# shenyunhang/APE

Hardware: AMD Instinct MI355X
Metric: images/sec @1024^2 APE-L_D fwd (higher is better)
Workload: dtype bf16

## Files before the change

ape_amd/_lib.py:

```python
import ctypes
import os
from ctypes import POINTER, Structure, c_char_p, c_double, c_float, c_int, c_int32, c_int64, c_void_p

_HERE = os.path.dirname(os.path.abspath(__file__))
LIB_PATH = os.path.join(_HERE, "lib", "libape_hip.so")

DT_F32 = 0
DT_BF16 = 1
DT_F16 = 2
ACT_NONE, ACT_RELU, ACT_GELU, ACT_SWIGLU, ACT_SILU = 0, 1, 2, 3, 4
MASK_NONE, MASK_ZERO_INPUT, MASK_ZERO_OUTPUT = 0, 1, 2


class GemmArgs(Structure):
    _fields_ = [
        ("A", c_void_p), ("W", c_void_p), ("C", c_void_p), ("bias", c_void_p), ("residual", c_void_p),
        ("rowmask", c_void_p), ("rope_cos", c_void_p), ("rope_sin", c_void_p),
        ("M", c_int32), ("N", c_int32), ("K", c_int32),
        ("lda", c_int32), ("ldw", c_int32), ("ldc", c_int32), ("ldr", c_int32),
        ("in_dt", c_int32), ("out_dt", c_int32), ("res_dt", c_int32),
        ("act", c_int32), ("mask_mode", c_int32), ("trans_out", c_int32),
        ("rope_rows", c_int32), ("rope_hd", c_int32), ("rope_cols", c_int32), ("vec_ok", c_int32),
        ("alpha", c_float), ("clamp", c_float),
        ("splitk", c_int32), ("tile64", c_int32), ("workspace", c_void_p),
# ... 98 lines not shown
    "ape_hip_query_init": (c_int, [c_void_p, c_void_p, c_int, c_void_p, c_int, c_float, c_int, c_void_p, c_void_p, c_int, c_int, c_void_p,
                                   c_void_p]),
    "ape_hip_query_finish": (c_int, [c_void_p, c_int, c_void_p, c_int, c_int, c_int, c_void_p, c_void_p, c_float, c_void_p, c_void_p,
                                     c_float, c_void_p, c_void_p, c_void_p, c_int, c_int, c_void_p]),
    "ape_hip_bilinear_resize": (c_int, [c_void_p, c_int, c_int, c_int, c_int, c_int, c_void_p, c_int, c_int, c_void_p]),
    "ape_hip_panoptic_pixels": (c_int, [c_void_p, c_int, c_int, c_int, c_int, c_int, c_void_p, c_void_p, c_float, c_int, c_int, c_void_p, c_void_p,
                                        c_void_p, c_void_p]),
    "ape_hip_panoptic_decide": (c_int, [c_void_p, c_void_p, c_void_p, c_int, c_void_p, c_int, c_double, c_int, c_void_p, c_void_p, c_void_p, c_void_p]),
    "ape_hip_panoptic_write": (c_int, [c_void_p, c_void_p, c_void_p, c_int, c_int, c_void_p, c_void_p]),
    "ape_hip_enc_finalize": (c_int, [c_void_p, c_void_p, c_void_p, c_int, c_void_p, c_void_p, c_void_p, c_void_p]),
    "ape_hip_topk_workspace_words": (c_int, [c_int]),
    "ape_hip_proposal_topk": (c_int, [c_void_p, c_int, POINTER(c_int), POINTER(c_int), c_int, c_int, c_int, c_void_p, c_void_p, c_void_p,
                                      c_void_p]),
    "ape_hip_proposal_order": (c_int, [c_void_p, c_int, c_void_p, c_void_p, POINTER(c_int), POINTER(c_int), c_int, c_void_p, c_void_p,
                                       c_void_p, c_void_p, c_void_p, c_void_p, c_void_p]),
    "ape_hip_proposal_quota": (c_int, [c_void_p, c_void_p, c_void_p, c_void_p, c_int, c_void_p, c_int, POINTER(c_int), POINTER(c_int),
                                       c_int, c_int, c_void_p, c_void_p]),
    "ape_hip_det_sort": (c_int, [c_void_p, c_int, c_int, c_int, c_void_p, c_void_p, c_float, c_void_p, c_void_p, c_void_p, c_void_p,
                                 c_void_p, c_void_p]),
    "ape_hip_det_topk": (c_int, [c_void_p, c_void_p, c_void_p, c_void_p, c_int, c_int, c_int, c_void_p, c_void_p, c_void_p, c_void_p,
                                 c_void_p, c_void_p]),
    "ape_hip_ffn_fused": (c_int, [c_void_p, c_int, c_void_p, c_int, c_void_p, c_void_p, c_int, c_void_p, c_void_p, c_int, c_void_p, c_int,
                                  c_int, c_int, c_int, c_int, c_int, c_int, c_void_p, c_void_p, c_float, c_void_p]),
    "ape_hip_attention_ext": (c_int, [c_void_p, c_int, c_void_p, c_int, c_void_p, c_int, c_void_p, c_int, c_int, c_int, c_int, c_int, c_int,
                                      c_int, c_float, c_int, c_void_p]),
    "ape_hip_relpos_extend": (c_int, [c_void_p, c_void_p, c_int, c_void_p, c_int, c_int, c_void_p, c_void_p, c_int, c_void_p, c_void_p, c_int, c_int,
                                      c_int, c_int, c_int, c_int, c_int, c_int, c_float, c_int, c_void_p]),
    "ape_hip_resize_coeffs": (c_int, [c_int, c_int, c_void_p, c_void_p, c_int]),
    "ape_hip_resize_tile_rows": (c_int, [c_void_p, c_int, POINTER(c_int)]),
    "ape_hip_resize_bilinear_u8": (c_int, [c_void_p, c_int, c_int, c_int, c_void_p, c_void_p, c_int, c_void_p, c_void_p, c_int,
                                           c_int, c_int, c_int, c_int, c_void_p, c_int, c_int, c_int, c_int, c_void_p]),
    "ape_hip_rle_workspace_words": (c_int, [c_int, c_int, c_int, c_int]),
    "ape_hip_rle_encode": (c_int, [c_void_p, c_int, c_int, c_int, c_void_p, c_void_p, c_int, c_void_p, c_void_p]),
    "ape_hip_rle_to_string": (c_int, [c_void_p, c_int, c_void_p, c_int]),
    "ape_hip_label_hist_lds_bins": (c_int, []),
    "ape_hip_label_pair_hist": (c_int, [c_void_p, c_int, c_void_p, c_int, ctypes.c_size_t, c_int, c_int, c_int, c_int, c_void_p, c_void_p,
                                        c_void_p]),
    "ape_hip_mask_pack_bits": (c_int, [c_void_p, c_int, ctypes.c_size_t, ctypes.c_size_t, c_void_p, ctypes.c_size_t, c_void_p, c_void_p]),
    "ape_hip_mask_paired_counts": (c_int, [c_void_p, ctypes.c_size_t, c_void_p, ctypes.c_size_t, c_int, ctypes.c_size_t, c_void_p, c_void_p]),
    "ape_hip_bitmask_pair_counts": (c_int, [c_void_p, c_int, ctypes.c_size_t, c_void_p, c_int, ctypes.c_size_t, ctypes.c_size_t, c_void_p,
                                            ctypes.c_size_t, c_void_p]),
    "ape_hip_rle_decode_workspace_words": (c_int, [c_int, c_int]),
    "ape_hip_rle_decode": (c_int, [c_void_p, c_void_p, c_int, c_int, c_int, c_int, c_void_p, c_void_p, c_void_p]),
    "ape_hip_rle_from_string": (c_int, [c_void_p, c_int, c_void_p, c_int]),
    "ape_hip_mask_pack_rows": (c_int, [c_void_p, c_int, c_int, c_int, c_void_p, ctypes.c_size_t, c_void_p, c_void_p]),
    "ape_hip_bitmask_boundary": (c_int, [c_void_p, c_int, c_int, c_int, c_int, ctypes.c_size_t, c_void_p, ctypes.c_size_t, c_void_p,
# ... 35 lines not shown
```

ape_amd/csrc/ffn_fused.hip:

```cpp
#include <stdlib.h>

#include "common.h"
#include "../../include/ape_hip.h"

typedef __attribute__((address_space(3))) void ff_lds_void_t;
typedef const __attribute__((address_space(1))) void ff_gbl_void_t;

#define FF_K 256
#define FF_HC 64
#define FF_N 256
#define FF_BM 128
#define FF_STAGE 65536

struct FfnParams {
  const bf16_t* X; int ldx;
  const bf16_t* W1; int ldw1;
  const float* b1;
  const bf16_t* W2; int ldw2;
  const float* b2;
  const bf16_t* R; int ldr;
  bf16_t* Y; int ldy;
  int M, HID;
  const float* ln_w; const float* ln_b; float ln_eps;
};

__device__ __forceinline__ float ff_rows_sum(float v) {
  const unsigned u = __float_as_uint(v);
  const auto a = __builtin_amdgcn_permlane16_swap(u, u, false, false);
  const float m = __uint_as_float(a[0]) + __uint_as_float(a[1]);
  const unsigned w = __float_as_uint(m);
  const auto b = __builtin_amdgcn_permlane32_swap(w, w, false, false);
  return __uint_as_float(b[0]) + __uint_as_float(b[1]);
}

template <bool W2P, int RT, typename H = bf16_t>
__global__ __launch_bounds__(256, 1) void ffn_fused_kernel(const FfnParams p) {
  extern __shared__ __attribute__((aligned(16))) unsigned char smem[];
  float* sb1 = reinterpret_cast<float*>(smem + 2 * FF_STAGE);
  float* sb2 = sb1 + p.HID;
  const int tid = threadIdx.x, lane = tid & 63, wave = tid >> 6;
  const int fm = lane & 15, g = lane >> 4;
  const int row0 = blockIdx.x * (64 * RT) + wave * (16 * RT);

  for (int i = tid; i < p.HID; i += 256) sb1[i] = p.b1[i];
  for (int i = tid; i < FF_N; i += 256) sb2[i] = p.b2[i];

  bf16x8_t xf[RT][8];
  int tok[RT];
#pragma unroll
  for (int rt = 0; rt < RT; ++rt) {
    tok[rt] = row0 + rt * 16 + fm;
    const bf16_t* xp = p.X + (size_t)(tok[rt] < p.M ? tok[rt] : p.M - 1) * p.ldx + g * 8;
#pragma unroll
    for (int ks = 0; ks < 8; ++ks) xf[rt][ks] = __builtin_bit_cast(bf16x8_t, *reinterpret_cast<const short8_t*>(xp + ks * 32));
  }

  uint32_t w1off[8], w2off[8];
#pragma unroll
// ... 125 lines not shown
#define FF_DMA(J) issue_piece(cn, s ^ 1, (J)); FF_SB();
    rd1(0, fa); rd1(1, fb); FF_SB();
    rd1(2, fc); mm1(0, fa); FF_MIX(8); FF_SB(); FF_DMA(0)
    rd1(3, fa); act(0); mm1(1, fb); FF_MIX(8); FF_SB(); FF_DMA(1)
    rd2(0, 0, fb); act(1); pack(0); mm1(2, fc); FF_MIX(8); FF_SB(); FF_DMA(2)
    rd2(0, 1, fc); act(2); mm1(3, fa); FF_MIX(8); FF_SB(); FF_DMA(3)
    rd2(1, 0, fa); act(3); pack(1); mm2(0, 0, fb); FF_MIX(8); FF_SB(); FF_DMA(4)
    rd2(1, 1, fb); mm2(0, 1, fc); FF_MIX(8); FF_SB(); FF_DMA(5)
    mm2(1, 0, fa); FF_SB(); FF_DMA(6)
    FF_DMA(7)
    mm2(1, 1, fb); FF_SB();
#undef FF_DMA
#undef FF_MIX
#undef FF_SB
    asm volatile("s_waitcnt vmcnt(0)" ::: "memory");
    __syncthreads();
  }

#pragma unroll
  for (int rt = 0; rt < RT; ++rt) {
    const int tk = tok[rt] < p.M ? tok[rt] : p.M - 1;
    const bf16_t* rp = p.R != nullptr ? p.R + (size_t)tk * p.ldr + g * 8 : nullptr;
    float v[64];
#pragma unroll
    for (int q = 0; q < 8; ++q) {
      const float4 ba = *reinterpret_cast<const float4*>(sb2 + q * 32 + g * 8);
      const float4 bb = *reinterpret_cast<const float4*>(sb2 + q * 32 + g * 8 + 4);
      v[q * 8 + 0] = yacc[2 * q][rt][0] + ba.x; v[q * 8 + 1] = yacc[2 * q][rt][1] + ba.y;
      v[q * 8 + 2] = yacc[2 * q][rt][2] + ba.z; v[q * 8 + 3] = yacc[2 * q][rt][3] + ba.w;
      v[q * 8 + 4] = yacc[2 * q + 1][rt][0] + bb.x; v[q * 8 + 5] = yacc[2 * q + 1][rt][1] + bb.y;
      v[q * 8 + 6] = yacc[2 * q + 1][rt][2] + bb.z; v[q * 8 + 7] = yacc[2 * q + 1][rt][3] + bb.w;
      if (rp != nullptr) {
        float r[8];
        ld8<H>(reinterpret_cast<const H*>(rp + q * 32), r);
#pragma unroll
        for (int e = 0; e < 8; ++e) v[q * 8 + e] += r[e];
      }
    }
    if (p.ln_w != nullptr) {
      float sum = 0.f;
#pragma unroll
      for (int e = 0; e < 64; ++e) sum += v[e];
      const float mean = ff_rows_sum(sum) * (1.f / FF_N);
      float d2 = 0.f;
#pragma unroll
      for (int e = 0; e < 64; ++e) { v[e] -= mean; d2 = fmaf(v[e], v[e], d2); }
      const float rstd = rsqrtf(ff_rows_sum(d2) * (1.f / FF_N) + p.ln_eps);
#pragma unroll
      for (int q = 0; q < 16; ++q) {
        const float4 w = *reinterpret_cast<const float4*>(p.ln_w + (q >> 1) * 32 + g * 8 + (q & 1) * 4);
        const float4 b = *reinterpret_cast<const float4*>(p.ln_b + (q >> 1) * 32 + g * 8 + (q & 1) * 4);
        v[q * 4 + 0] = fmaf(v[q * 4 + 0] * rstd, w.x, b.x); v[q * 4 + 1] = fmaf(v[q * 4 + 1] * rstd, w.y, b.y);
        v[q * 4 + 2] = fmaf(v[q * 4 + 2] * rstd, w.z, b.z); v[q * 4 + 3] = fmaf(v[q * 4 + 3] * rstd, w.w, b.w);
      }
    }
    if (tok[rt] < p.M) {
      bf16_t* yp = p.Y + (size_t)tok[rt] * p.ldy + g * 8;
#pragma unroll
      for (int q = 0; q < 8; ++q) st8<H>(reinterpret_cast<H*>(yp + q * 32), v + q * 8);
    }
  }
}

extern "C" int ape_hip_ffn_fused(const void* X, int ldx, const void* W1, int ldw1, const float* b1, const void* W2, int ldw2, const float* b2,
                                 const void* residual, int ldr, void* Y, int ldy, int M, int K, int HID, int N, int w2_permuted, int dt,
                                 const float* ln_weight, const float* ln_bias, float ln_eps, void* stream) {
  APE_CHECK_ARG(X && W1 && b1 && W2 && b2 && Y && M > 0, "ape_hip_ffn_fused: null pointer / empty problem");
  APE_CHECK_ARG(ape_is16(dt), "ape_hip_ffn_fused: dt must be APE_DT_BF16 or APE_DT_F16 (got %d)", dt);
  APE_CHECK_ARG(K == FF_K && N == FF_N && HID % FF_HC == 0 && HID >= FF_HC && HID <= 4096,
                "ape_hip_ffn_fused: the kernel is built for 256 -> HID -> 256 with HID %% 64 == 0, HID <= 4096 (got %d -> %d -> %d)", K, HID, N);
  APE_CHECK_ARG(ldx % 8 == 0 && ldw1 % 8 == 0 && ldw2 % 8 == 0 && ldy % 8 == 0 && (residual == nullptr || ldr % 8 == 0),
                "ape_hip_ffn_fused: leading dimensions must be multiples of 8");
  APE_CHECK_ARG(((uintptr_t)X) % 16 == 0 && ((uintptr_t)W1) % 16 == 0 && ((uintptr_t)W2) % 16 == 0 && ((uintptr_t)Y) % 16 == 0 &&
                    ((uintptr_t)residual) % 16 == 0 && ((uintptr_t)b1) % 16 == 0 && ((uintptr_t)b2) % 16 == 0,
                "ape_hip_ffn_fused: 16-byte aligned pointers");
  APE_CHECK_ARG((size_t)HID * ldw1 * 2 < (1ull << 32) && (size_t)FF_N * ldw2 * 2 < (1ull << 32), "ape_hip_ffn_fused: weights too large for 32-bit offsets");
  FfnParams p;
  p.X = (const bf16_t*)X; p.ldx = ldx; p.W1 = (const bf16_t*)W1; p.ldw1 = ldw1; p.b1 = b1; p.W2 = (const bf16_t*)W2; p.ldw2 = ldw2; p.b2 = b2;
  p.R = (const bf16_t*)residual; p.ldr = ldr; p.Y = (bf16_t*)Y; p.ldy = ldy; p.M = M; p.HID = HID;
  APE_CHECK_ARG((ln_weight == nullptr) == (ln_bias == nullptr) && ((uintptr_t)ln_weight) % 16 == 0 && ((uintptr_t)ln_bias) % 16 == 0,
                "ape_hip_ffn_fused: LayerNorm weight and bias come together, 16-byte aligned");
  p.ln_w = ln_weight; p.ln_b = ln_bias; p.ln_eps = ln_eps;
  const size_t lds = 2 * FF_STAGE + (size_t)(HID + FF_N) * sizeof(float);
  const char* rt_env = getenv("APE_FFN_RT");
  const int rt = rt_env != nullptr ? atoi(rt_env) : (ceil_div(M, 192) >= 256 ? 3 : 2);
#define FF_LAUNCH(W2P_, RT_, H_)                                                                                              \
  do {                                                                                                                        \
    static ApeOncePerDevice attr__;                                                                                               \
    if (attr__.first()) {                                                                                                            \
      (void)hipFuncSetAttribute((const void*)ffn_fused_kernel<W2P_, RT_, H_>, hipFuncAttributeMaxDynamicSharedMemorySize, 160 * 1024); \
    }                                                                                                                         \
    APE_LAUNCH((ffn_fused_kernel<W2P_, RT_, H_>), dim3(ceil_div(M, 64 * RT_)), dim3(256), lds, (hipStream_t)stream, p); \
  } while (0)
  if (dt == APE_DT_F16) {
    if (w2_permuted && rt == 3) FF_LAUNCH(true, 3, f16_t); else if (w2_permuted) FF_LAUNCH(true, 2, f16_t); else FF_LAUNCH(false, 2, f16_t);
  } else {
    if (w2_permuted && rt == 3) FF_LAUNCH(true, 3, bf16_t); else if (w2_permuted) FF_LAUNCH(true, 2, bf16_t); else FF_LAUNCH(false, 2, bf16_t);
  }
#undef FF_LAUNCH
  APE_CHECK_LAUNCH("ffn_fused_kernel");
  return 0;
}
```

ape_amd/layers/fuse_helper.py:

```python
import torch
import torch.nn as nn

from .. import ops
from ..packing import attach_cache, f32, ln_params, pack_matrix


class BiMultiHeadAttention(nn.Module):
    def __init__(self, v_dim, l_dim, embed_dim, num_heads, dropout=0.1, stable_softmax_2d=False,
                 clamp_min_for_underflow=True, clamp_max_for_overflow=True, use_attention_mask_v=False):
        super().__init__()
        self.embed_dim, self.num_heads, self.head_dim = embed_dim, num_heads, embed_dim // num_heads
        self.v_dim, self.l_dim = v_dim, l_dim
        assert self.head_dim * num_heads == embed_dim
        self.scale = self.head_dim ** (-0.5)
        self.dropout = dropout
        self.v_proj = nn.Linear(v_dim, embed_dim)
        self.l_proj = nn.Linear(l_dim, embed_dim)
        self.values_v_proj = nn.Linear(v_dim, embed_dim)
        self.values_l_proj = nn.Linear(l_dim, embed_dim)
        self.out_v_proj = nn.Linear(embed_dim, v_dim)
        self.out_l_proj = nn.Linear(embed_dim, l_dim)
        self.stable_softmax_2d = stable_softmax_2d
        self.clamp_min_for_underflow = clamp_min_for_underflow
        self.clamp_max_for_overflow = clamp_max_for_overflow
# ... 70 lines not shown
        gmax = S.max().reshape(1)
        pv = ops.segment_softmax(S, nh, gmax, dt)
        v_new = ops.gemm(pv, Zt, Pd["bov"], residual=v_n, out_dtype=dt)
        qp = v_new + lvl_pos
        plT = ops.col_softmax_t(S, gmax, dt, pad=8)
        vT = ops.transpose(v_n, pad=8)
        G = ops.gemm(plT, vT, None, out_dtype=dt)
        ol = torch.empty((L, nh * hd), dtype=dt, device=dev)
        for h in range(nh):
            ops.gemm(G[h * L:(h + 1) * L], Pd["wvv"][h], Pd["bvv"][h], out=ol[:, h * hd:(h + 1) * hd])
        dl = ops.gemm(ol, Pd["wol"], Pd["bol"], out_dtype=torch.float32)
        l_new = l_n + P["gl"] * dl
        return v_new, qp, l_new

    def forward_tokens(self, x, lvl_pos, l, dt, defer_language=False):
        if l.shape[0] == 1:
            v_new, qp, ljob = self.forward_tokens_single(x, lvl_pos, l, dt)
        else:
            v_new, qp, l_new = self.forward_tokens_dense(x, lvl_pos, l, dt)
            ljob = ops._Joined(l_new)
        return (v_new, qp, ljob) if defer_language else (v_new, qp, ljob.join())

    def forward_tokens_single(self, x, lvl_pos, l, dt):
        P = self.packed(dt)
        a = self.attn
        l_n = ops.layernorm(l, P["lnl"][0], P["lnl"][1], P["lnl"][2], out_dtype=torch.float32)
        k = ops.gemv(l_n, P["wl"], P["bl"])
        vl = ops.gemv(l_n, P["wvl"], P["bvl"])
        gdv, lnb = ops.gemv(vl, P["wov"], P["bov"], scale=P["gv"], add=P["lnv"][1][None, :])
        v_new, qp = ops.layernorm(x, P["lnv"][0], lnb[0], P["lnv"][2], out_dtype=dt, add=lvl_pos)

        def language_side():
            kh = k.view(a.num_heads, a.head_dim)
            u, u_c = ops.head_gemv(kh, P["wvT"], bf16_copy=dt if dt in ops.HALF16 else True)
            c = ops.head_gemv(kh, P["bv1"], alpha=a.scale)
            _, sbias = ops.gemv(gdv, u, alpha=-a.scale, add=c.view(1, -1))
            S = ops.gemm(v_new, u_c if dt in ops.HALF16 else u, sbias[0], alpha=a.scale, out_dtype=torch.float32)
            pooled = ops.vl_pool(S, v_new, gdv[0])
            ol = ops.head_gemv(pooled, P["wvv"], P["bvv"])
            return ops.gemv(ol.view(1, -1), P["wol"], P["bol"], scale=P["gl"], add=l_n)[1]

        return v_new, qp, ops.fork(language_side)

    def forward(self, v, l, attention_mask_v=None, attention_mask_l=None):
        if attention_mask_l is not None:
            raise NotImplementedError("ape_amd BiAttentionBlock: per-token language masks (un-reduced expression tokens, "
                                      "text_feature_reduce_before_fusion=False) are not implemented")
        dt = getattr(self, "compute_dtype", torch.bfloat16)
        vs, ls = [], []
        for b in range(v.shape[0]):
            zeros = torch.zeros_like(v[b], dtype=dt)
            vn, _, ln = self.forward_tokens(v[b].to(dt).contiguous(), zeros, l[b].float().contiguous(), dt)
            vs.append(vn.to(v.dtype))
            ls.append(ln.to(l.dtype))
        return torch.stack(vs), torch.stack(ls)
```

ape_amd/modeling/ape_deta/_containers.py:

```python
import os

import torch
import torch.nn as nn

from ... import ops
from ...packing import attach_cache, f32, ln_params, pack_matrix, permute_ffn_w2


class FFN(nn.Module):
    def __init__(self, embed_dim=256, feedforward_dim=1024, output_dim=None, num_fcs=2, ffn_drop=0.0, **kwargs):
        super().__init__()
        assert num_fcs == 2
        output_dim = embed_dim if output_dim is None else output_dim
        self.layers = nn.Sequential(nn.Sequential(nn.Linear(embed_dim, feedforward_dim), nn.ReLU(inplace=True), nn.Dropout(ffn_drop)),
                                    nn.Linear(feedforward_dim, output_dim), nn.Dropout(ffn_drop))
        self.embed_dim = embed_dim
        attach_cache(self)

    def packed(self, dt):
        def build(dt):
            l0, l1 = self.layers[0][0], self.layers[1]
            d = dict(w1=pack_matrix(l0.weight, dt), b1=f32(l0.bias), w2=pack_matrix(l1.weight, dt), b2=f32(l1.bias))
            if dt in ops.HALF16 and l0.weight.shape[0] % 64 == 0:
                d["w2p"] = permute_ffn_w2(d["w2"])
            return d
        return self._pack.get(self, dt, build)

    FUSED_MIN_ROWS = 2048

    def forward_tokens(self, x, dt, out_dtype=None, norm=None):
        P = self.packed(dt)
        mode = os.environ.get("APE_FFN_FUSED", "1")
        if (mode != "0" and "w2p" in P and (out_dtype or dt) in ops.HALF16 and (out_dtype or dt) == dt and x.shape[0] >= self.FUSED_MIN_ROWS
                and x.shape[1] == 256 and P["w2"].shape[0] == 256 and P["w1"].shape[0] <= 4096):
            fuse_ln = norm if os.environ.get("APE_FFN_LN") != "0" else None
            if mode == "b64":
                y = ops.ffn_fused(x, P["w1"], P["b1"], P["w2"], P["b2"], residual=x, norm=fuse_ln)
            else:
                y = ops.ffn_fused(x, P["w1"], P["b1"], P["w2p"], P["b2"], residual=x, w2_permuted=True, norm=fuse_ln)
            return y if (norm is None or fuse_ln is not None) else ops.layernorm(y, norm[0], norm[1], norm[2], out_dtype=dt)
        h = ops.gemm(x, P["w1"], P["b1"], act=ops.ACT_RELU)
        y = ops.gemm(h, P["w2"], P["b2"], residual=x, out_dtype=out_dtype or dt)
        return y if norm is None else ops.layernorm(y, norm[0], norm[1], norm[2], out_dtype=dt)


class MLP(nn.Module):
    def __init__(self, input_dim, hidden_dim, output_dim, num_layers):
        super().__init__()
        self.num_layers = num_layers
        h = [hidden_dim] * (num_layers - 1)
        self.layers = nn.ModuleList(nn.Linear(n, k) for n, k in zip([input_dim] + h, h + [output_dim]))
        attach_cache(self)

    def packed(self, dt):
        def build(dt):
            return [(pack_matrix(l.weight, dt), f32(l.bias)) for l in self.layers]
        return self._pack.get(self, dt, build)
# ... 78 lines not shown
```

ape_amd/modeling/ape_deta/deformable_transformer_vl.py:

```python
import copy

import torch
import torch.nn as nn

from ... import ops
from ...layers import MultiScaleDeformableAttention
from ...packing import attach_cache, f32, ln_params, pack_matrix, round_up
from ...stagetap import forcing, tap
from . import geometry as G
from ._containers import FFN, SelfAttention, TransformerLayer


class DeformableDetrTransformerEncoderVL(nn.Module):
    def __init__(self, embed_dim=256, num_heads=8, feedforward_dim=1024, attn_dropout=0.1, ffn_dropout=0.1, num_layers=6,
                 post_norm=False, num_feature_levels=4, vl_layer=None, use_act_checkpoint=False, pytorch_attn=False):
        super().__init__()
        self.layers = nn.ModuleList([
            TransformerLayer([MultiScaleDeformableAttention(embed_dim=embed_dim, num_heads=num_heads, dropout=attn_dropout,
                                                            batch_first=True, num_levels=num_feature_levels,
                                                            pytorch_attn=pytorch_attn)],
                             FFN(embed_dim=embed_dim, feedforward_dim=feedforward_dim, output_dim=embed_dim, num_fcs=2,
                                 ffn_drop=ffn_dropout), 2, embed_dim) for _ in range(num_layers)])
        self.num_layers = num_layers
        self.embed_dim = embed_dim
        self.pre_norm = False
        self.post_norm_layer = nn.LayerNorm(embed_dim) if post_norm else None
        self.vl_layers = nn.ModuleList([copy.deepcopy(vl_layer) for _ in range(num_layers)]) if vl_layer is not None else None
        self.use_checkpoint = use_act_checkpoint

    def forward_tokens(self, x, geo, lvl_pos, l, dt, stages=None):
        xp = None
        for i, layer in enumerate(self.layers):
            if self.vl_layers is None:
                v_new, qp, ljob = x, (xp if xp is not None else (x.float() + lvl_pos.float()).to(dt)), ops._Joined(l)
            else:
                v_new, qp, ljob = self.vl_layers[i].b_attn.forward_tokens(x, lvl_pos, l, dt, defer_language=True)
            x2 = layer.attentions[0].forward_tokens(qp, v_new, geo.enc_ref, geo.shapes, geo.starts, dt, value_src=v_new,
                                                    mask=geo.mask_u8, norm=layer.norm_params(0))
            x, xp = layer.ffns[0].forward_tokens(x2, dt, norm=layer.norm_params(1)), None
            l = ljob.join()
            if stages is not None:
                if self.vl_layers is not None:
                    stages[f"enc{i}_fused_v"] = v_new
                    l = tap(stages, f"enc{i}_fused_l", l)
                x = tap(stages, f"enc{i}_out", x)
        if self.post_norm_layer is not None:
            x = ops.layernorm(x, *ln_params(self.post_norm_layer), out_dtype=dt)
        return x, l


class DeformableDetrTransformerDecoderVL(nn.Module):
    def __init__(self, embed_dim=256, num_heads=8, feedforward_dim=1024, attn_dropout=0.1, ffn_dropout=0.1, num_layers=6,
                 return_intermediate=True, num_feature_levels=4, use_act_checkpoint=False, look_forward_twice=False,
                 pytorch_attn=False):
        super().__init__()
        self.layers = nn.ModuleList([
            TransformerLayer([SelfAttention(embed_dim=embed_dim, num_heads=num_heads, attn_drop=attn_dropout, batch_first=True),
                              MultiScaleDeformableAttention(embed_dim=embed_dim, num_heads=num_heads, dropout=attn_dropout,
                                                            batch_first=True, num_levels=num_feature_levels,
                                                            pytorch_attn=pytorch_attn)],
                             FFN(embed_dim=embed_dim, feedforward_dim=feedforward_dim, output_dim=embed_dim, ffn_drop=ffn_dropout),
                             3, embed_dim) for _ in range(num_layers)])
        self.num_layers = num_layers
        self.embed_dim = embed_dim
        self.return_intermediate = return_intermediate
        self.bbox_embed = None
        self.class_embed = None
        self.use_checkpoint = use_act_checkpoint
# ... 189 lines not shown
```

ape_amd/ops.py:

```python
import ctypes
import math
import os

import numpy as np
import torch

from . import _lib
from ._lib import (ACT_GELU, ACT_NONE, ACT_RELU, ACT_SILU, ACT_SWIGLU, DT_BF16, DT_F32, MASK_NONE,
                   MASK_ZERO_INPUT, MASK_ZERO_OUTPUT)

_DT = {torch.float32: DT_F32, torch.bfloat16: DT_BF16, torch.float16: _lib.DT_F16}
HALF16 = (torch.bfloat16, torch.float16)


def _dt(t):
    try:
        return _DT[t.dtype]
    except KeyError:
        raise TypeError(f"ape_amd: unsupported dtype {t.dtype} (float32 / bfloat16 / float16 only)")


def _dev(*ts):
    for t in ts:
        if t is not None and not t.is_cuda:
# ... 1452 lines not shown
        raise TypeError("ape_amd.ops.detections: logits must be float32")
    _f32c(boxes, "boxes", (Q, 4)), _f32c(scale, "scale", (4,))
    dev = logits.device
    lib = _lib.load()
    xyxy = torch.empty((Q, 4), dtype=torch.float32, device=dev)
    finite = torch.empty((Q,), dtype=torch.uint8, device=dev)
    sorted_scores = torch.empty((K, Q), dtype=torch.float32, device=dev)
    order = torch.empty((K, Q), dtype=torch.int32, device=dev)
    valid = torch.empty((K, Q), dtype=torch.uint8, device=dev)
    rc = lib.ape_hip_det_sort(_p(logits), _ld(logits), Q, K, _p(boxes), _p(scale), float(score_thresh), _p(xyxy), _p(finite),
                              _p(sorted_scores), _p(order), _p(valid), _stream())
    _lib.check(rc, "ape_hip_det_sort")
    keep = nms_classes(xyxy, order, iou_thr, valid)
    k = min(int(topk), K * Q)
    det = dict(det_boxes=torch.empty((k, 4), dtype=torch.float32, device=dev), det_scores=torch.empty((k,), dtype=torch.float32, device=dev),
               det_classes=torch.empty((k,), dtype=torch.int64, device=dev), det_query=torch.empty((k,), dtype=torch.int64, device=dev))
    ws = torch.empty((lib.ape_hip_topk_workspace_words(K * Q),), dtype=torch.int64, device=dev)
    rc = lib.ape_hip_det_topk(_p(sorted_scores), _p(keep), _p(order), _p(xyxy), K, Q, k, _p(ws), _p(det["det_boxes"]), _p(det["det_scores"]),
                              _p(det["det_classes"]), _p(det["det_query"]), _stream())
    _lib.check(rc, "ape_hip_det_topk")
    return det


def ffn_fused(x, w1, b1, w2, b2, residual=None, out=None, w2_permuted=False, norm=None):
    _dev(x, w1, w2, b1, b2, residual, out)
    for t, name in ((x, "x"), (w1, "w1"), (w2, "w2")):
        _rowmajor(t, name)
        if t.dtype not in HALF16 or t.dtype != x.dtype:
            raise TypeError(f"ape_amd.ops.ffn_fused: {name} must be bfloat16 or float16, one type per call")
    M, K = x.shape
    HID, N = w1.shape[0], w2.shape[0]
    if w1.shape[1] != K or w2.shape[1] != HID:
        raise ValueError("ape_amd.ops.ffn_fused: weight shapes do not chain")
    if out is None:
        out = torch.empty((M, N), dtype=x.dtype, device=x.device)
    if out.dtype != x.dtype:
        raise TypeError("ape_amd.ops.ffn_fused: out must have x's dtype")
    if residual is not None:
        _rowmajor(residual, "residual")
        if residual.dtype != x.dtype or tuple(residual.shape) != (M, N):
            raise TypeError("ape_amd.ops.ffn_fused: residual must be [M, N] in x's dtype")
    if norm is not None:
        _dev(norm[0], norm[1])
        if norm[0].numel() != N or norm[1].numel() != N:
            raise ValueError("ape_amd.ops.ffn_fused: norm = (weight [N], bias [N], eps)")
    rc = _lib.load().ape_hip_ffn_fused(_p(x), _ld(x), _p(w1), _ld(w1), _p(_f32vec(b1, "b1")), _p(w2), _ld(w2), _p(_f32vec(b2, "b2")),
                                      _p(residual), _ld(residual) if residual is not None else 0, _p(out), _ld(out), M, K, HID, N,
                                      1 if w2_permuted else 0, _dt(x), _p(_f32vec(norm[0], "norm weight")) if norm is not None else None,
                                      _p(_f32vec(norm[1], "norm bias")) if norm is not None else None,
                                      float(norm[2]) if norm is not None else 0.0, _stream())
    _lib.check(rc, "ape_hip_ffn_fused")
    return out
```

include/ape_hip.h:

```cpp
#ifndef APE_HIP_H
#define APE_HIP_H
#include <stdint.h>

#ifdef __cplusplus
extern "C" {
#endif

#define APE_DT_F32 0
#define APE_DT_BF16 1
#define APE_DT_F16 2

#define APE_ACT_NONE 0
#define APE_ACT_RELU 1
#define APE_ACT_GELU 2
#define APE_ACT_SWIGLU 3
#define APE_ACT_SILU 4

#define APE_MASK_NONE 0
#define APE_MASK_ZERO_INPUT 1
#define APE_MASK_ZERO_OUTPUT 2

const char* ape_hip_last_error(void);
int ape_hip_abi_version(void);
int ape_hip_sizeof_args(int which);
// ... 194 lines not shown
int ape_hip_topk_workspace_words(int n_total);
int ape_hip_proposal_topk(const float* logit, int T, const int* level_start, const int* level_n, int L, int k, int k_alt,
                          uint64_t* workspace, int32_t* cand, int32_t* alt, void* stream);
int ape_hip_proposal_order(const int32_t* cand, int n, const float* logit, const float* xyxy, const int* level_start,
                           const int* level_n, int L, float* boxes_b, int32_t* groups_b, int32_t* seg, int32_t* cand_a,
                           int32_t* lv_a, int32_t* pos_b, void* stream);
int ape_hip_proposal_quota(const int32_t* cand_a, const int32_t* lv_a, const int32_t* pos_b, const uint8_t* keep_b, int n,
                           const int32_t* alt, int n_alt, const int* level_start, const int* level_n, int L, int nq, int64_t* out,
                           void* stream);
int ape_hip_det_sort(const float* logits, int ldl, int Q, int K, const float* boxes, const float* scale, float thresh, float* xyxy,
                     uint8_t* finite, float* sorted, int32_t* order, uint8_t* valid, void* stream);
int ape_hip_det_topk(const float* sorted, const uint8_t* keep, const int32_t* order, const float* xyxy, int K, int Q, int k,
                     uint64_t* workspace, float* det_boxes, float* det_scores, int64_t* det_classes, int64_t* det_query, void* stream);

int ape_hip_attention_ext(const void* Q, int ldq, const void* K, int ldk, const void* Vt, int ldvt, void* O, int ldo, int B, int N,
                          int bstride, int H, int HDQ, int HDV, float scale, int dt, void* stream);
int ape_hip_relpos_extend(const void* q, const void* k, int ldqk, const void* t, int ldt, int tper, const int* ty, const int* tx, int period,
                          void* q_ext, void* k_ext, int lde, int rows, int nh, int hs, int hd, int Hk, int Wk, int hdq, float scale, int dt,
                          void* stream);

int ape_hip_ffn_fused(const void* X, int ldx, const void* W1, int ldw1, const float* b1, const void* W2, int ldw2, const float* b2,
                      const void* residual, int ldr, void* Y, int ldy, int M, int K, int HID, int N, int w2_permuted, int dt,
                      const float* ln_weight, const float* ln_bias, float ln_eps, void* stream);

int ape_hip_label_hist_lds_bins(void);
int ape_hip_label_pair_hist(const void* a, int a_bytes, const void* b, int b_bytes, size_t n, int na, int nb, int a_ignore,
                            int b_ignore, int64_t* hist, int64_t* rejected, void* stream);

int ape_hip_mask_pack_bits(const uint8_t* masks, int n, size_t npix, size_t stride, uint64_t* bits, size_t ldb, int64_t* area,
                           void* stream);
int ape_hip_mask_paired_counts(const uint8_t* a, size_t stride_a, const uint8_t* b, size_t stride_b, int n, size_t npix, int64_t* out,
                               void* stream);
int ape_hip_bitmask_pair_counts(const uint64_t* a, int n, size_t lda, const uint64_t* b, int m, size_t ldb, size_t words,
                                int64_t* inter, size_t ldi, void* stream);
int ape_hip_rle_decode_workspace_words(int n, int cap);
int ape_hip_rle_decode(const uint32_t* counts, const uint32_t* nruns, int n, int cap, int H, int W, uint32_t* workspace,
                       uint8_t* masks, void* stream);
int ape_hip_rle_from_string(const char* s, int len, uint32_t* counts, int cap);

int ape_hip_mask_pack_rows(const uint8_t* masks, int n, int H, int W, uint64_t* bits, size_t ldb, int64_t* area, void* stream);
int ape_hip_bitmask_boundary(const uint64_t* bits, int n, int H, int W, int d, size_t ldb, uint64_t* bbits, size_t ldo, int64_t* barea,
                             void* stream);
int ape_hip_bitmask_boundary_tile(int H, int W, int d, size_t lds_limit, int* tile_rows, int* tile_words);
int ape_hip_bitmask_unpack_rows(const uint64_t* bits, int n, int H, int W, size_t ldb, uint8_t* masks, void* stream);

int ape_hip_box_cover_overlaps(const float* proposals, int n, const float* gt, const float* gt_area, int m, const float* ranges,
// ... 12 lines not shown
```

Measured before the change: 114.5.

## Fuse next layer's vision LayerNorm and pos-add into encoder FFN epilogue

Adds a chained variant of the fused FFN kernel whose epilogue, after the post-FFN LayerNorm, also applies the next encoder layer's vision LayerNorm and adds the level position embedding. It writes both the normalized value and the query input. The encoder loop is restructured so that the language-side work and the next layer's language prologue run in a forked branch, joined before the FFN that needs its bias. This removes a separate LayerNorm launch and a full activation read and write per encoder layer. In exchange it adds register pressure in the epilogue and an extra bf16 store stream.

```diff
diff --git a/ape_amd/_lib.py b/ape_amd/_lib.py
--- a/ape_amd/_lib.py
+++ b/ape_amd/_lib.py
@@ -144,6 +144,9 @@
                                  c_void_p, c_void_p]),
     "ape_hip_ffn_fused": (c_int, [c_void_p, c_int, c_void_p, c_int, c_void_p, c_void_p, c_int, c_void_p, c_void_p, c_int, c_void_p, c_int,
                                   c_int, c_int, c_int, c_int, c_int, c_int, c_void_p, c_void_p, c_float, c_void_p]),
+    "ape_hip_ffn_fused_chain": (c_int, [c_void_p, c_int, c_void_p, c_int, c_void_p, c_void_p, c_int, c_void_p, c_void_p, c_int, c_void_p, c_int,
+                                        c_int, c_int, c_int, c_int, c_int, c_int, c_void_p, c_void_p, c_float, c_void_p, c_void_p, c_float,
+                                        c_void_p, c_int, c_void_p, c_int, c_void_p]),
     "ape_hip_attention_ext": (c_int, [c_void_p, c_int, c_void_p, c_int, c_void_p, c_int, c_void_p, c_int, c_int, c_int, c_int, c_int, c_int,
                                       c_int, c_float, c_int, c_void_p]),
     "ape_hip_relpos_extend": (c_int, [c_void_p, c_void_p, c_int, c_void_p, c_int, c_int, c_void_p, c_void_p, c_int, c_void_p, c_void_p, c_int, c_int,
diff --git a/ape_amd/csrc/ffn_fused.hip b/ape_amd/csrc/ffn_fused.hip
--- a/ape_amd/csrc/ffn_fused.hip
+++ b/ape_amd/csrc/ffn_fused.hip
@@ -22,6 +22,9 @@
   bf16_t* Y; int ldy;
   int M, HID;
   const float* ln_w; const float* ln_b; float ln_eps;
+  const float* ln2_w; const float* ln2_b; float ln2_eps;
+  const bf16_t* add; int ldadd;
+  bf16_t* Y2; int ldy2;
 };
 
 __device__ __forceinline__ float ff_rows_sum(float v) {
@@ -33,7 +36,24 @@
   return __uint_as_float(b[0]) + __uint_as_float(b[1]);
 }
 
-template <bool W2P, int RT, typename H = bf16_t>
+__device__ __forceinline__ float ff_rows_sum_ln(const float (&part)[16]) {
+  float c[2];
+#pragma unroll
+  for (int h = 0; h < 2; ++h) {
+    const float a0 = part[0 + h] + part[8 + h], a1 = part[2 + h] + part[10 + h], a2 = part[4 + h] + part[12 + h], a3 = part[6 + h] + part[14 + h];
+    const float b0 = a0 + a2, b1 = a1 + a3;
+    const float s = b0 + b1;
+    const unsigned u = __float_as_uint(s);
+    const auto x = __builtin_amdgcn_permlane32_swap(u, u, false, false);
+    const float m = __uint_as_float(x[0]) + __uint_as_float(x[1]);
+    const unsigned w = __float_as_uint(m);
+    const auto y = __builtin_amdgcn_permlane16_swap(w, w, false, false);
+    c[h] = __uint_as_float(y[0]) + __uint_as_float(y[1]);
+  }
+  return c[0] + c[1];
+}
+
+template <bool W2P, int RT, typename H = bf16_t, bool CHAIN = false>
 __global__ __launch_bounds__(256, 1) void ffn_fused_kernel(const FfnParams p) {
   extern __shared__ __attribute__((aligned(16))) unsigned char smem[];
   float* sb1 = reinterpret_cast<float*>(smem + 2 * FF_STAGE);
@@ -205,6 +225,12 @@
     const int tk = tok[rt] < p.M ? tok[rt] : p.M - 1;
     const bf16_t* rp = p.R != nullptr ? p.R + (size_t)tk * p.ldr + g * 8 : nullptr;
     float v[64];
+    uint4 araw[CHAIN ? 8 : 1];
+    if constexpr (CHAIN) {
+      const bf16_t* ap = p.add + (size_t)tk * p.ldadd + g * 8;
+#pragma unroll
+      for (int q = 0; q < 8; ++q) araw[q] = *reinterpret_cast<const uint4*>(ap + q * 32);
+    }
 #pragma unroll
     for (int q = 0; q < 8; ++q) {
       const float4 ba = *reinterpret_cast<const float4*>(sb2 + q * 32 + g * 8);
@@ -220,7 +246,7 @@
         for (int e = 0; e < 8; ++e) v[q * 8 + e] += r[e];
       }
     }
-    if (p.ln_w != nullptr) {
+    if (CHAIN || p.ln_w != nullptr) {
       float sum = 0.f;
 #pragma unroll
       for (int e = 0; e < 64; ++e) sum += v[e];
@@ -237,7 +263,39 @@
         v[q * 4 + 2] = fmaf(v[q * 4 + 2] * rstd, w.z, b.z); v[q * 4 + 3] = fmaf(v[q * 4 + 3] * rstd, w.w, b.w);
       }
     }
-    if (tok[rt] < p.M) {
+    if constexpr (CHAIN) {
+#pragma unroll
+      for (int e = 0; e < 64; e += 2) unpack2<H>(h16<H>::pack2(v[e], v[e + 1]), v[e], v[e + 1]);
+      float part[16];
+#pragma unroll
+      for (int j = 0; j < 16; ++j) part[j] = (v[4 * j] + v[4 * j + 1]) + (v[4 * j + 2] + v[4 * j + 3]);
+      const float mean = ff_rows_sum_ln(part) * (1.f / FF_N);
+#pragma unroll
+      for (int j = 0; j < 16; ++j) {
+        float d2 = 0.f;
+#pragma unroll
+        for (int r = 0; r < 4; ++r) { v[4 * j + r] -= mean; d2 = fmaf(v[4 * j + r], v[4 * j + r], d2); }
+        part[j] = d2;
+      }
+      const float rstd = rsqrtf(ff_rows_sum_ln(part) * (1.f / FF_N) + p.ln2_eps);
+      const bool live = tok[rt] < p.M;
+      bf16_t* yp = p.Y + (size_t)tk * p.ldy + g * 8;
+      bf16_t* y2p = p.Y2 + (size_t)tk * p.ldy2 + g * 8;
+#pragma unroll
+      for (int q = 0; q < 8; ++q) {
+        const float4 wa = *reinterpret_cast<const float4*>(p.ln2_w + q * 32 + g * 8), wb = *reinterpret_cast<const float4*>(p.ln2_w + q * 32 + g * 8 + 4);
+        const float4 ba = *reinterpret_cast<const float4*>(p.ln2_b + q * 32 + g * 8), bb = *reinterpret_cast<const float4*>(p.ln2_b + q * 32 + g * 8 + 4);
+        const float w[8] = {wa.x, wa.y, wa.z, wa.w, wb.x, wb.y, wb.z, wb.w}, b[8] = {ba.x, ba.y, ba.z, ba.w, bb.x, bb.y, bb.z, bb.w};
+        float a[8], o[8];
+        unpack2<H>(araw[q].x, a[0], a[1]); unpack2<H>(araw[q].y, a[2], a[3]); unpack2<H>(araw[q].z, a[4], a[5]); unpack2<H>(araw[q].w, a[6], a[7]);
+#pragma unroll
+        for (int e = 0; e < 8; ++e) { o[e] = fmaf(v[q * 8 + e] * rstd, w[e], b[e]); a[e] += o[e]; }
+        if (live) {
+          st8<H>(reinterpret_cast<H*>(yp + q * 32), o);
+          st8<H>(reinterpret_cast<H*>(y2p + q * 32), a);
+        }
+      }
+    } else if (tok[rt] < p.M) {
       bf16_t* yp = p.Y + (size_t)tok[rt] * p.ldy + g * 8;
 #pragma unroll
       for (int q = 0; q < 8; ++q) st8<H>(reinterpret_cast<H*>(yp + q * 32), v + q * 8);
@@ -245,42 +303,76 @@
   }
 }
 
-extern "C" int ape_hip_ffn_fused(const void* X, int ldx, const void* W1, int ldw1, const float* b1, const void* W2, int ldw2, const float* b2,
-                                 const void* residual, int ldr, void* Y, int ldy, int M, int K, int HID, int N, int w2_permuted, int dt,
-                                 const float* ln_weight, const float* ln_bias, float ln_eps, void* stream) {
-  APE_CHECK_ARG(X && W1 && b1 && W2 && b2 && Y && M > 0, "ape_hip_ffn_fused: null pointer / empty problem");
-  APE_CHECK_ARG(ape_is16(dt), "ape_hip_ffn_fused: dt must be APE_DT_BF16 or APE_DT_F16 (got %d)", dt);
+static int ffn_fused_run(const char* who, const void* X, int ldx, const void* W1, int ldw1, const float* b1, const void* W2, int ldw2, const float* b2,
+                         const void* residual, int ldr, void* Y, int ldy, int M, int K, int HID, int N, int w2_permuted, int dt,
+                         const float* ln_weight, const float* ln_bias, float ln_eps, bool chain, const float* ln2_weight, const float* ln2_bias,
+                         float ln2_eps, const void* add, int ldadd, void* Y2, int ldy2, void* stream) {
+  APE_CHECK_ARG(X && W1 && b1 && W2 && b2 && Y && M > 0, "%s: null pointer / empty problem", who);
+  APE_CHECK_ARG(ape_is16(dt), "%s: dt must be APE_DT_BF16 or APE_DT_F16 (got %d)", who, dt);
   APE_CHECK_ARG(K == FF_K && N == FF_N && HID % FF_HC == 0 && HID >= FF_HC && HID <= 4096,
-                "ape_hip_ffn_fused: the kernel is built for 256 -> HID -> 256 with HID %% 64 == 0, HID <= 4096 (got %d -> %d -> %d)", K, HID, N);
+                "%s: the kernel is built for 256 -> HID -> 256 with HID %% 64 == 0, HID <= 4096 (got %d -> %d -> %d)", who, K, HID, N);
   APE_CHECK_ARG(ldx % 8 == 0 && ldw1 % 8 == 0 && ldw2 % 8 == 0 && ldy % 8 == 0 && (residual == nullptr || ldr % 8 == 0),
-                "ape_hip_ffn_fused: leading dimensions must be multiples of 8");
+                "%s: leading dimensions must be multiples of 8", who);
   APE_CHECK_ARG(((uintptr_t)X) % 16 == 0 && ((uintptr_t)W1) % 16 == 0 && ((uintptr_t)W2) % 16 == 0 && ((uintptr_t)Y) % 16 == 0 &&
                     ((uintptr_t)residual) % 16 == 0 && ((uintptr_t)b1) % 16 == 0 && ((uintptr_t)b2) % 16 == 0,
-                "ape_hip_ffn_fused: 16-byte aligned pointers");
-  APE_CHECK_ARG((size_t)HID * ldw1 * 2 < (1ull << 32) && (size_t)FF_N * ldw2 * 2 < (1ull << 32), "ape_hip_ffn_fused: weights too large for 32-bit offsets");
+                "%s: 16-byte aligned pointers", who);
+  APE_CHECK_ARG((size_t)HID * ldw1 * 2 < (1ull << 32) && (size_t)FF_N * ldw2 * 2 < (1ull << 32), "%s: weights too large for 32-bit offsets", who);
   FfnParams p;
   p.X = (const bf16_t*)X; p.ldx = ldx; p.W1 = (const bf16_t*)W1; p.ldw1 = ldw1; p.b1 = b1; p.W2 = (const bf16_t*)W2; p.ldw2 = ldw2; p.b2 = b2;
   p.R = (const bf16_t*)residual; p.ldr = ldr; p.Y = (bf16_t*)Y; p.ldy = ldy; p.M = M; p.HID = HID;
   APE_CHECK_ARG((ln_weight == nullptr) == (ln_bias == nullptr) && ((uintptr_t)ln_weight) % 16 == 0 && ((uintptr_t)ln_bias) % 16 == 0,
-                "ape_hip_ffn_fused: LayerNorm weight and bias come together, 16-byte aligned");
+                "%s: LayerNorm weight and bias come together, 16-byte aligned", who);
   p.ln_w = ln_weight; p.ln_b = ln_bias; p.ln_eps = ln_eps;
+  p.ln2_w = nullptr; p.ln2_b = nullptr; p.ln2_eps = 0.f; p.add = nullptr; p.ldadd = 0; p.Y2 = nullptr; p.ldy2 = 0;
+  if (chain) {
+    APE_CHECK_ARG(ln_weight != nullptr, "%s: the chained LayerNorm follows the first one (ln_weight / ln_bias are required)", who);
+    APE_CHECK_ARG(ln2_weight != nullptr && ln2_bias != nullptr, "%s: ln2_weight and ln2_bias are required", who);
+    APE_CHECK_ARG(((uintptr_t)ln2_weight) % 16 == 0 && ((uintptr_t)ln2_bias) % 16 == 0, "%s: ln2_weight / ln2_bias must be 16-byte aligned", who);
+    APE_CHECK_ARG(add != nullptr && Y2 != nullptr, "%s: add and Y2 go together and are both required", who);
+    APE_CHECK_ARG(ldadd % 8 == 0 && ldy2 % 8 == 0 && ldadd >= FF_N && ldy2 >= FF_N, "%s: ldadd / ldy2 must be multiples of 8, at least 256", who);
+    APE_CHECK_ARG(((uintptr_t)add) % 16 == 0 && ((uintptr_t)Y2) % 16 == 0, "%s: add / Y2 must be 16-byte aligned", who);
+    APE_CHECK_ARG(w2_permuted != 0, "%s: the chained kernel is built for the pre-permuted W2 only", who);
+    p.ln2_w = ln2_weight; p.ln2_b = ln2_bias; p.ln2_eps = ln2_eps; p.add = (const bf16_t*)add; p.ldadd = ldadd; p.Y2 = (bf16_t*)Y2; p.ldy2 = ldy2;
+  }
   const size_t lds = 2 * FF_STAGE + (size_t)(HID + FF_N) * sizeof(float);
   const char* rt_env = getenv("APE_FFN_RT");
   const int rt = rt_env != nullptr ? atoi(rt_env) : (ceil_div(M, 192) >= 256 ? 3 : 2);
-#define FF_LAUNCH(W2P_, RT_, H_)                                                                                              \
+#define FF_LAUNCH(RT_, ...)                                                                                                    \
   do {                                                                                                                        \
-    static ApeOncePerDevice attr__;                                                                                               \
-    if (attr__.first()) {                                                                                                            \
-      (void)hipFuncSetAttribute((const void*)ffn_fused_kernel<W2P_, RT_, H_>, hipFuncAttributeMaxDynamicSharedMemorySize, 160 * 1024); \
+    static ApeOncePerDevice attr__;                                                                                           \
+    if (attr__.first()) {                                                                                                     \
+      (void)hipFuncSetAttribute((const void*)__VA_ARGS__, hipFuncAttributeMaxDynamicSharedMemorySize, 160 * 1024);            \
     }                                                                                                                         \
-    APE_LAUNCH((ffn_fused_kernel<W2P_, RT_, H_>), dim3(ceil_div(M, 64 * RT_)), dim3(256), lds, (hipStream_t)stream, p); \
+    APE_LAUNCH((__VA_ARGS__), dim3(ceil_div(M, 64 * RT_)), dim3(256), lds, (hipStream_t)stream, p);                           \
   } while (0)
-  if (dt == APE_DT_F16) {
-    if (w2_permuted && rt == 3) FF_LAUNCH(true, 3, f16_t); else if (w2_permuted) FF_LAUNCH(true, 2, f16_t); else FF_LAUNCH(false, 2, f16_t);
+  if (chain) {
+    if (dt == APE_DT_F16) { if (rt == 3) FF_LAUNCH(3, ffn_fused_kernel<true, 3, f16_t, true>); else FF_LAUNCH(2, ffn_fused_kernel<true, 2, f16_t, true>); }
+    else { if (rt == 3) FF_LAUNCH(3, ffn_fused_kernel<true, 3, bf16_t, true>); else FF_LAUNCH(2, ffn_fused_kernel<true, 2, bf16_t, true>); }
+  } else if (dt == APE_DT_F16) {
+    if (w2_permuted && rt == 3) FF_LAUNCH(3, ffn_fused_kernel<true, 3, f16_t>);
+    else if (w2_permuted) FF_LAUNCH(2, ffn_fused_kernel<true, 2, f16_t>);
+    else FF_LAUNCH(2, ffn_fused_kernel<false, 2, f16_t>);
   } else {
-    if (w2_permuted && rt == 3) FF_LAUNCH(true, 3, bf16_t); else if (w2_permuted) FF_LAUNCH(true, 2, bf16_t); else FF_LAUNCH(false, 2, bf16_t);
+    if (w2_permuted && rt == 3) FF_LAUNCH(3, ffn_fused_kernel<true, 3, bf16_t>);
+    else if (w2_permuted) FF_LAUNCH(2, ffn_fused_kernel<true, 2, bf16_t>);
+    else FF_LAUNCH(2, ffn_fused_kernel<false, 2, bf16_t>);
   }
 #undef FF_LAUNCH
   APE_CHECK_LAUNCH("ffn_fused_kernel");
   return 0;
 }
+
+extern "C" int ape_hip_ffn_fused(const void* X, int ldx, const void* W1, int ldw1, const float* b1, const void* W2, int ldw2, const float* b2,
+                                 const void* residual, int ldr, void* Y, int ldy, int M, int K, int HID, int N, int w2_permuted, int dt,
+                                 const float* ln_weight, const float* ln_bias, float ln_eps, void* stream) {
+  return ffn_fused_run("ape_hip_ffn_fused", X, ldx, W1, ldw1, b1, W2, ldw2, b2, residual, ldr, Y, ldy, M, K, HID, N, w2_permuted, dt, ln_weight, ln_bias,
+                       ln_eps, false, nullptr, nullptr, 0.f, nullptr, 0, nullptr, 0, stream);
+}
+
+extern "C" int ape_hip_ffn_fused_chain(const void* X, int ldx, const void* W1, int ldw1, const float* b1, const void* W2, int ldw2, const float* b2,
+                                       const void* residual, int ldr, void* Y, int ldy, int M, int K, int HID, int N, int w2_permuted, int dt,
+                                       const float* ln_weight, const float* ln_bias, float ln_eps, const float* ln2_weight, const float* ln2_bias,
+                                       float ln2_eps, const void* add, int ldadd, void* Y2, int ldy2, void* stream) {
+  return ffn_fused_run("ape_hip_ffn_fused_chain", X, ldx, W1, ldw1, b1, W2, ldw2, b2, residual, ldr, Y, ldy, M, K, HID, N, w2_permuted, dt, ln_weight,
+                       ln_bias, ln_eps, true, ln2_weight, ln2_bias, ln2_eps, add, ldadd, Y2, ldy2, stream);
+}
diff --git a/ape_amd/layers/fuse_helper.py b/ape_amd/layers/fuse_helper.py
--- a/ape_amd/layers/fuse_helper.py
+++ b/ape_amd/layers/fuse_helper.py
@@ -116,25 +116,38 @@
         return (v_new, qp, ljob) if defer_language else (v_new, qp, ljob.join())
 
     def forward_tokens_single(self, x, lvl_pos, l, dt):
+        pro = self.language_prologue(l, dt)
+        v_new, qp = self.vision_norm(x, lvl_pos, pro, dt)
+        return v_new, qp, ops.fork(lambda: self.language_side(v_new, pro, dt))
+
+    def language_prologue(self, l, dt):
         P = self.packed(dt)
-        a = self.attn
         l_n = ops.layernorm(l, P["lnl"][0], P["lnl"][1], P["lnl"][2], out_dtype=torch.float32)
         k = ops.gemv(l_n, P["wl"], P["bl"])
         vl = ops.gemv(l_n, P["wvl"], P["bvl"])
         gdv, lnb = ops.gemv(vl, P["wov"], P["bov"], scale=P["gv"], add=P["lnv"][1][None, :])
-        v_new, qp = ops.layernorm(x, P["lnv"][0], lnb[0], P["lnv"][2], out_dtype=dt, add=lvl_pos)
+        return l_n, k, gdv, lnb
 
-        def language_side():
-            kh = k.view(a.num_heads, a.head_dim)
-            u, u_c = ops.head_gemv(kh, P["wvT"], bf16_copy=dt if dt in ops.HALF16 else True)
-            c = ops.head_gemv(kh, P["bv1"], alpha=a.scale)
-            _, sbias = ops.gemv(gdv, u, alpha=-a.scale, add=c.view(1, -1))
-            S = ops.gemm(v_new, u_c if dt in ops.HALF16 else u, sbias[0], alpha=a.scale, out_dtype=torch.float32)
-            pooled = ops.vl_pool(S, v_new, gdv[0])
-            ol = ops.head_gemv(pooled, P["wvv"], P["bvv"])
-            return ops.gemv(ol.view(1, -1), P["wol"], P["bol"], scale=P["gl"], add=l_n)[1]
+    def vision_norm_params(self, pro, dt):
+        P = self.packed(dt)
+        return P["lnv"][0], pro[3][0], P["lnv"][2]
 
-        return v_new, qp, ops.fork(language_side)
+    def vision_norm(self, x, lvl_pos, pro, dt):
+        w, b, eps = self.vision_norm_params(pro, dt)
+        return ops.layernorm(x, w, b, eps, out_dtype=dt, add=lvl_pos)
+
+    def language_side(self, v_new, pro, dt):
+        P = self.packed(dt)
+        a = self.attn
+        l_n, k, gdv, _ = pro
+        kh = k.view(a.num_heads, a.head_dim)
+        u, u_c = ops.head_gemv(kh, P["wvT"], bf16_copy=dt if dt in ops.HALF16 else True)
+        c = ops.head_gemv(kh, P["bv1"], alpha=a.scale)
+        _, sbias = ops.gemv(gdv, u, alpha=-a.scale, add=c.view(1, -1))
+        S = ops.gemm(v_new, u_c if dt in ops.HALF16 else u, sbias[0], alpha=a.scale, out_dtype=torch.float32)
+        pooled = ops.vl_pool(S, v_new, gdv[0])
+        ol = ops.head_gemv(pooled, P["wvv"], P["bvv"])
+        return ops.gemv(ol.view(1, -1), P["wol"], P["bol"], scale=P["gl"], add=l_n)[1]
 
     def forward(self, v, l, attention_mask_v=None, attention_mask_l=None):
         if attention_mask_l is not None:
diff --git a/ape_amd/modeling/ape_deta/_containers.py b/ape_amd/modeling/ape_deta/_containers.py
--- a/ape_amd/modeling/ape_deta/_containers.py
+++ b/ape_amd/modeling/ape_deta/_containers.py
@@ -28,11 +28,28 @@
 
     FUSED_MIN_ROWS = 2048
 
-    def forward_tokens(self, x, dt, out_dtype=None, norm=None):
+    @staticmethod
+    def chain_in_kernel(x):
+        return x.is_cuda
+
+    def _one_kernel(self, x, dt, out_dtype):
+        P = self.packed(dt)
+        return (os.environ.get("APE_FFN_FUSED", "1") != "0" and "w2p" in P and (out_dtype or dt) in ops.HALF16 and (out_dtype or dt) == dt
+                and x.shape[0] >= self.FUSED_MIN_ROWS and x.shape[1] == 256 and P["w2"].shape[0] == 256 and P["w1"].shape[0] <= 4096)
+
+    def forward_tokens(self, x, dt, out_dtype=None, norm=None, chain=None):
+        if chain is not None:
+            if norm is None:
+                raise ValueError("FFN.forward_tokens: chain follows the layer's post-FFN norm (norm is required)")
+            if (self._one_kernel(x, dt, out_dtype) and os.environ.get("APE_FFN_FUSED", "1") != "b64" and os.environ.get("APE_FFN_LN") != "0"
+                    and self.chain_in_kernel(x)):
+                P = self.packed(dt)
+                return ops.ffn_fused(x, P["w1"], P["b1"], P["w2p"], P["b2"], residual=x, w2_permuted=True, norm=norm, chain=chain)
+            y = self.forward_tokens(x, dt, out_dtype, norm)
+            return ops.layernorm(y, chain[0], chain[1], chain[2], out_dtype=dt, add=chain[3])
         P = self.packed(dt)
         mode = os.environ.get("APE_FFN_FUSED", "1")
-        if (mode != "0" and "w2p" in P and (out_dtype or dt) in ops.HALF16 and (out_dtype or dt) == dt and x.shape[0] >= self.FUSED_MIN_ROWS
-                and x.shape[1] == 256 and P["w2"].shape[0] == 256 and P["w1"].shape[0] <= 4096):
+        if self._one_kernel(x, dt, out_dtype):
             fuse_ln = norm if os.environ.get("APE_FFN_LN") != "0" else None
             if mode == "b64":
                 y = ops.ffn_fused(x, P["w1"], P["b1"], P["w2"], P["b2"], residual=x, norm=fuse_ln)
diff --git a/ape_amd/modeling/ape_deta/deformable_transformer_vl.py b/ape_amd/modeling/ape_deta/deformable_transformer_vl.py
--- a/ape_amd/modeling/ape_deta/deformable_transformer_vl.py
+++ b/ape_amd/modeling/ape_deta/deformable_transformer_vl.py
@@ -1,4 +1,5 @@
 import copy
+import os
 
 import torch
 import torch.nn as nn
@@ -29,6 +30,9 @@
         self.use_checkpoint = use_act_checkpoint
 
     def forward_tokens(self, x, geo, lvl_pos, l, dt, stages=None):
+        if (self.vl_layers is not None and l.shape[0] == 1 and stages is None and dt in ops.HALF16
+                and os.environ.get("APE_ENC_CHAIN") != "0"):
+            return self._forward_tokens_chained(x, geo, lvl_pos, l, dt)
         xp = None
         for i, layer in enumerate(self.layers):
             if self.vl_layers is None:
@@ -44,6 +48,29 @@
                     stages[f"enc{i}_fused_v"] = v_new
                     l = tap(stages, f"enc{i}_fused_l", l)
                 x = tap(stages, f"enc{i}_out", x)
+        if self.post_norm_layer is not None:
+            x = ops.layernorm(x, *ln_params(self.post_norm_layer), out_dtype=dt)
+        return x, l
+
+    def _forward_tokens_chained(self, x, geo, lvl_pos, l, dt):
+        blocks = [vl.b_attn for vl in self.vl_layers]
+        last = len(self.layers) - 1
+        pro = blocks[0].language_prologue(l, dt)
+        v_new, qp = blocks[0].vision_norm(x, lvl_pos, pro, dt)
+        for i, layer in enumerate(self.layers):
+            def branch(i=i, v_new=v_new, pro=pro):
+                l_new = blocks[i].language_side(v_new, pro, dt)
+                return l_new, (blocks[i + 1].language_prologue(l_new, dt) if i < last else None)
+            ljob = ops.fork(branch)
+            x2 = layer.attentions[0].forward_tokens(qp, v_new, geo.enc_ref, geo.shapes, geo.starts, dt, value_src=v_new,
+                                                    mask=geo.mask_u8, norm=layer.norm_params(0))
+            if i < last:
+                l, pro = ljob.join()
+                w, b, eps = blocks[i + 1].vision_norm_params(pro, dt)
+                v_new, qp = layer.ffns[0].forward_tokens(x2, dt, norm=layer.norm_params(1), chain=(w, b, eps, lvl_pos))
+            else:
+                x = layer.ffns[0].forward_tokens(x2, dt, norm=layer.norm_params(1))
+                l, _ = ljob.join()
         if self.post_norm_layer is not None:
             x = ops.layernorm(x, *ln_params(self.post_norm_layer), out_dtype=dt)
         return x, l
diff --git a/ape_amd/ops.py b/ape_amd/ops.py
--- a/ape_amd/ops.py
+++ b/ape_amd/ops.py
@@ -1498,7 +1498,7 @@
     return det
 
 
-def ffn_fused(x, w1, b1, w2, b2, residual=None, out=None, w2_permuted=False, norm=None):
+def ffn_fused(x, w1, b1, w2, b2, residual=None, out=None, w2_permuted=False, norm=None, chain=None, out2=None):
     _dev(x, w1, w2, b1, b2, residual, out)
     for t, name in ((x, "x"), (w1, "w1"), (w2, "w2")):
         _rowmajor(t, name)
@@ -1520,10 +1520,27 @@
         _dev(norm[0], norm[1])
         if norm[0].numel() != N or norm[1].numel() != N:
             raise ValueError("ape_amd.ops.ffn_fused: norm = (weight [N], bias [N], eps)")
-    rc = _lib.load().ape_hip_ffn_fused(_p(x), _ld(x), _p(w1), _ld(w1), _p(_f32vec(b1, "b1")), _p(w2), _ld(w2), _p(_f32vec(b2, "b2")),
-                                      _p(residual), _ld(residual) if residual is not None else 0, _p(out), _ld(out), M, K, HID, N,
-                                      1 if w2_permuted else 0, _dt(x), _p(_f32vec(norm[0], "norm weight")) if norm is not None else None,
-                                      _p(_f32vec(norm[1], "norm bias")) if norm is not None else None,
-                                      float(norm[2]) if norm is not None else 0.0, _stream())
-    _lib.check(rc, "ape_hip_ffn_fused")
-    return out
+    head = (_p(x), _ld(x), _p(w1), _ld(w1), _p(_f32vec(b1, "b1")), _p(w2), _ld(w2), _p(_f32vec(b2, "b2")),
+            _p(residual), _ld(residual) if residual is not None else 0, _p(out), _ld(out), M, K, HID, N,
+            1 if w2_permuted else 0, _dt(x), _p(_f32vec(norm[0], "norm weight")) if norm is not None else None,
+            _p(_f32vec(norm[1], "norm bias")) if norm is not None else None, float(norm[2]) if norm is not None else 0.0)
+    if chain is None:
+        _lib.check(_lib.load().ape_hip_ffn_fused(*head, _stream()), "ape_hip_ffn_fused")
+        return out
+    if norm is None:
+        raise ValueError("ape_amd.ops.ffn_fused: chain follows the first LayerNorm: norm = (weight, bias, eps) is required")
+    cw, cb, ceps, add = chain
+    _dev(cw, cb, add, out2)
+    if cw.numel() != N or cb.numel() != N:
+        raise ValueError("ape_amd.ops.ffn_fused: chain = (weight [N], bias [N], eps, add [M, N])")
+    _rowmajor(add, "add")
+    if add.dtype != x.dtype or tuple(add.shape) != (M, N):
+        raise TypeError("ape_amd.ops.ffn_fused: chain's add must be [M, N] in x's dtype")
+    if out2 is None:
+        out2 = torch.empty((M, N), dtype=x.dtype, device=x.device)
+    if out2.dtype != x.dtype or tuple(out2.shape) != (M, N):
+        raise TypeError("ape_amd.ops.ffn_fused: out2 must be [M, N] in x's dtype")
+    rc = _lib.load().ape_hip_ffn_fused_chain(*head, _p(_f32vec(cw, "chain weight")), _p(_f32vec(cb, "chain bias")), float(ceps),
+                                            _p(add), _ld(add), _p(_rowmajor(out2, "out2")), _ld(out2), _stream())
+    _lib.check(rc, "ape_hip_ffn_fused_chain")
+    return out, out2
diff --git a/include/ape_hip.h b/include/ape_hip.h
--- a/include/ape_hip.h
+++ b/include/ape_hip.h
@@ -240,6 +240,10 @@
 int ape_hip_ffn_fused(const void* X, int ldx, const void* W1, int ldw1, const float* b1, const void* W2, int ldw2, const float* b2,
                       const void* residual, int ldr, void* Y, int ldy, int M, int K, int HID, int N, int w2_permuted, int dt,
                       const float* ln_weight, const float* ln_bias, float ln_eps, void* stream);
+int ape_hip_ffn_fused_chain(const void* X, int ldx, const void* W1, int ldw1, const float* b1, const void* W2, int ldw2, const float* b2,
+                            const void* residual, int ldr, void* Y, int ldy, int M, int K, int HID, int N, int w2_permuted, int dt,
+                            const float* ln_weight, const float* ln_bias, float ln_eps, const float* ln2_weight, const float* ln2_bias,
+                            float ln2_eps, const void* add, int ldadd, void* Y2, int ldy2, void* stream);
 
 int ape_hip_label_hist_lds_bins(void);
 int ape_hip_label_pair_hist(const void* a, int a_bytes, const void* b, int b_bytes, size_t n, int na, int nb, int a_ignore,
```

Measured after the change: 114.3. Within noise of the previous version (-0.1%).
